# GerHobbelt/ugrep

Hardware: AMD Instinct MI355X
Metric: GB/s scanned + matches/s, 16 GiB synthetic buffer, 1/2/4/8 MI355X (higher is better)
Workload: dtype u8; 1 GPU; 3-literal alternation 'foo|bar|baz' over 16 GiB synthetic ASCII words; config=c2, pattern=foo|bar|baz, bytes_per_gpu=17179869184, total_bytes=17179869184, corpus_kind=1, parallelism=shard1, tables=reference, word=False, dfa_states=9, dfa_row=256, prefilter_ppm=4

## Files before the change

ugrep_amd/csrc/engine.hip:

```cpp
#include <hip/hip_runtime.h>

#include <cstdio>
#include <cstdlib>
#include <cstring>
#include <algorithm>
#include <atomic>
#include <chrono>
#include <condition_variable>
#include <deque>
#include <mutex>
#include <new>
#include <string>
#include <thread>
#include <future>
#include <vector>

#include "../../include/ugpu.h"
#include "plan.hpp"
#include "scan_kernels.hpp"
#include "tables.hpp"

ugpu::Utf8Params utf8_params(const uint8_t* dbuf, uint64_t len)
{
  static std::atomic<int> cached[64];
// ... 73 lines not shown
  bool word = false;
  bool wfast = false;
  bool wu = false;
  bool wforce = false;
  bool xu_exact = false;
  int word_rec = 0;
  bool wxc = false;
  uint32_t bol0 = 1;
  size_t smem = 0;
  size_t xi_smem = 0;
  int xi_rec = 0;
  bool last_xi = false;
  const uint8_t* last_buf = nullptr;
  uint64_t last_args[5] = {0, 0, 0, 0, 0};
  BlockRec* d_recs = nullptr;
  uint64_t* d_entries = nullptr;
  uint64_t* d_obase = nullptr;
  uint16_t* d_inbits = nullptr;
  uint64_t inbits_cap = 0;
  uint64_t* d_fix = nullptr;
  OpenRec* d_open = nullptr;
  uint32_t* d_susp = nullptr;
  SuspRec* d_srec = nullptr;
  DevTotals* d_tot = nullptr;
  uint32_t* d_flags = nullptr;
  DevTotals* h_tot = nullptr;
  uint32_t* h_flags = nullptr;
  hipEvent_t ev0 = nullptr, ev1 = nullptr;
  hipStream_t stream = nullptr;
  ScanParams last{};
  uint64_t off = 0;
  bool have_scan = false;
  bool forest = false;
  uint64_t f_cap = 0;
  uint32_t* d_fex = nullptr;
  uint64_t* d_fvar = nullptr;
  uint64_t* d_fent = nullptr;
  uint64_t* d_fsum = nullptr;
  uint64_t* d_fbase = nullptr;
  bool stage = false, stage_once = false, staged_last = false;
  uint64_t* d_st_start = nullptr;
  uint32_t* d_st_len = nullptr;
  uint32_t* d_st_cap = nullptr;
  uint32_t* d_st_n = nullptr;
};

namespace {

const char* const kBudgetMsg =
    "the FIND chains of this table do not resynchronise on this input (stitch budget exceeded): use the CPU matcher";
// ... 208 lines not shown
  if (pos == 0) pos = fb;
  if (pos > s->f_cap) {
    forest_free(s);
    const uint64_t nb = pos / fb;
    hipError_t e;
    if ((e = hipMalloc(&s->d_fex, pos * 4)) != hipSuccess || (e = hipMalloc(&s->d_fvar, 4 * 8)) != hipSuccess ||
        (e = hipMalloc(&s->d_fent, nb * 8)) != hipSuccess || (e = hipMalloc(&s->d_fsum, nb * 24)) != hipSuccess ||
        (e = hipMalloc(&s->d_fbase, nb * 8)) != hipSuccess) {
      forest_free(s);
      return hip_fail(e, "forest scratch");
    }
    s->f_cap = pos;
  }
  UGPU_TRACE("forest entry %llu hi %llu rend %llu write %d\n", (unsigned long long)entry,
             (unsigned long long)P.hi, (unsigned long long)P.rend, (int)write);
  ForestArgs A{};
  A.ex = s->d_fex;
  A.entry = s->d_fvar;
  A.run = s->d_fvar + 1;
  A.bentry = s->d_fent;
  A.bsum = s->d_fsum;
  A.bbase = s->d_fbase;
  P.flags = s->d_flags;
  HIP_TRY(hipMemsetAsync(s->d_flags, 0, sizeof(uint32_t), st));
  HIP_TRY(launch_forest(P, s->dfa->t.format, A, entry, write, s->d_tot, st));
  HIP_TRY(hipMemcpyAsync(s->h_tot, s->d_tot, sizeof(DevTotals), hipMemcpyDeviceToHost, st));
  HIP_TRY(hipMemcpyAsync(s->h_flags, s->d_flags, sizeof(uint32_t), hipMemcpyDeviceToHost, st));
  HIP_TRY(hipStreamSynchronize(st));
  return UGPU_OK;
}

int dfa_on(const ugpu_dfa* d, int dev, const ugpu_dfa** out);

}

extern "C" {

int ugpu_device_count(int* n)
{
  if (!n) return fail(UGPU_INVAL, "NULL argument");
  *n = 0;
  HIP_TRY(hipGetDeviceCount(n));
  exit_guard_arm();
  return UGPU_OK;
}

// ... 259 lines not shown
      return fail(UGPU_UNSUPPORTED, "tables do not fit in LDS");
    }
    s->word = true;
    s->word_rec = kMaxRec;
    if (const char* env = std::getenv("UGPU_MAX_GRID")) {
      int v = std::atoi(env);
      if (v >= 1 && v <= kMaxRec) s->word_rec = v;
    }
    s->max_rec = s->word_rec;
  }
  if (s->word && dfa->wplus) {
    s->word = false;
    s->wfast = true;
  } else if (s->word && dfa->xcw) {
    s->word = false;
    s->wxc = true;
  }
  if (s->word) {
    HIP_TRY_S(hipMalloc(&s->d_recs, sizeof(BlockRec) * kMaxRec));
    HIP_TRY_S(hipMalloc(&s->d_entries, sizeof(uint64_t) * kMaxRec));
    HIP_TRY_S(hipMalloc(&s->d_obase, sizeof(uint64_t) * kMaxRec));
    HIP_TRY_S(hipMalloc(&s->d_fix, sizeof(uint64_t) * kMaxRec));
    HIP_TRY_S(hipMalloc(&s->d_tot, sizeof(DevTotals)));
    HIP_TRY_S(hipMalloc(&s->d_flags, sizeof(uint32_t)));
    HIP_TRY_S(hipHostMalloc(&s->h_tot, sizeof(DevTotals)));
    HIP_TRY_S(hipHostMalloc(&s->h_flags, sizeof(uint32_t)));
    HIP_TRY_S(hipEventCreate(&s->ev0));
    HIP_TRY_S(hipEventCreate(&s->ev1));
    *out = s;
    return UGPU_OK;
  }
  const char* senv = std::getenv("UGPU_SPARSE");
  s->sparse = (dfa->t.filter || dfa->lb || dfa->wsparse) && dfa->t.format == FMT_BYTE && !(senv && senv[0] == '0');
  s->smem = s->sparse ? sparse_smem_bytes(dfa->ntrans_pad, dfa->t.states, acap_lds_n(dfa))
                      : dense_smem_bytes(dfa->t.format, dfa->ntrans_pad, dfa->t.states);
  if (s->smem > 160 * 1024) {
    delete s;
    return fail(UGPU_UNSUPPORTED, "tables do not fit in LDS");
  }
  int per_cu = 0;
  if (s->sparse) {
    ScanParams probe{};
    HIP_TRY_S(sparse_occupancy(probe, s->smem, &per_cu));
  } else {
    HIP_TRY_S(dense_occupancy(dfa->t.format, dfa->t.cap1 != 0, dfa->d_xtrans != nullptr, s->smem, &per_cu));
  }
  hipDeviceProp_t prop;
  HIP_TRY_S(hipGetDeviceProperties(&prop, s->device));
  if (per_cu < 1) per_cu = 1;
// ... 44 lines not shown
    if (cpc >= 1) {
      s->xc = true;
      s->xu = xu;
      s->wu = wu;
      s->xu_xi = s->xi;
      s->xu_xg = s->xg;
      s->xi = s->xg = false;
      const int cg = prop.multiProcessorCount * cpc * (int)xc_waves();
      s->xi_rec = cg > kMaxRec ? kMaxRec : cg;
      if (const char* env = std::getenv("UGPU_MAX_GRID")) {
        int v = std::atoi(env);
        if (v >= 1 && v <= kMaxRec) s->xi_rec = v;
      }
    }
  }
  HIP_TRY_S(hipMalloc(&s->d_recs, sizeof(BlockRec) * kMaxRec));
  HIP_TRY_S(hipMalloc(&s->d_entries, sizeof(uint64_t) * kMaxRec));
  HIP_TRY_S(hipMalloc(&s->d_obase, sizeof(uint64_t) * kMaxRec));
  HIP_TRY_S(hipMalloc(&s->d_fix, sizeof(uint64_t) * kMaxRec));
  if (s->sparse) {
    HIP_TRY_S(hipMalloc(&s->d_open, sizeof(OpenRec) * kMaxRec));
    HIP_TRY_S(hipMalloc(&s->d_susp, sizeof(uint32_t) * kMaxRec));
    HIP_TRY_S(hipMalloc(&s->d_srec, sizeof(SuspRec) * kMaxRec));
  }
  HIP_TRY_S(hipMalloc(&s->d_tot, sizeof(DevTotals)));
  HIP_TRY_S(hipMalloc(&s->d_flags, sizeof(uint32_t)));
  HIP_TRY_S(hipHostMalloc(&s->h_tot, sizeof(DevTotals)));
  HIP_TRY_S(hipHostMalloc(&s->h_flags, sizeof(uint32_t)));
  HIP_TRY_S(hipEventCreate(&s->ev0));
  HIP_TRY_S(hipEventCreate(&s->ev1));
  *out = s;
  return UGPU_OK;
#undef HIP_TRY_S
}

}

int ugpu_scanner_destroy(ugpu_scanner* s)
{
  if (!s || exiting()) return UGPU_OK;
  (void)hipFree(s->d_recs);
  (void)hipFree(s->d_entries);
  (void)hipFree(s->d_obase);
  (void)hipFree(s->d_inbits);
  (void)hipFree(s->d_fix);
  (void)hipFree(s->d_open);
  (void)hipFree(s->d_susp);
  (void)hipFree(s->d_srec);
  (void)hipFree(s->d_tot);
  (void)hipFree(s->d_flags);
  (void)hipHostFree(s->h_tot);
  (void)hipHostFree(s->h_flags);
  forest_free(s);
  (void)hipFree(s->d_st_start);
  (void)hipFree(s->d_st_len);
  (void)hipFree(s->d_st_cap);
  (void)hipFree(s->d_st_n);
  if (s->ev0) (void)hipEventDestroy(s->ev0);
  if (s->ev1) (void)hipEventDestroy(s->ev1);
  delete s;
  return UGPU_OK;
}

int ugpu_scan(ugpu_scanner* s, const uint8_t* dbuf, uint64_t lo, uint64_t hi, uint64_t read_end, int at_eof,
              uint64_t bias, void* stream)
{
  if (!s || !dbuf) return fail(UGPU_INVAL, "NULL argument");
  if (lo > hi || hi > read_end) return fail(UGPU_INVAL, "need lo <= hi <= read_end");
  hipStream_t st = reinterpret_cast<hipStream_t>(stream);
  if (s->wxc) s->word = false;
  if (s->wfast) {
// ... 12 lines not shown
    }
    s->word = !fast;
  }
  ScanParams P{};
  fill_tables(P, s->dfa);
  P.xu_tab = s->xu ? s->dfa->d_xu : nullptr;
  P.xu_w = s->wu && !s->word ? 1u : 0u;
  P.xu_exact = s->xu_exact ? 1u : 0u;
  P.bol0 = s->bol0;
  if (s->wfast && !s->word) P.wtab = nullptr, P.nwtab = 0;
  geometry_for(P, s, dbuf, lo, hi, read_end, s->off, s->xi || s->xg || s->xc);
  P.delta = (int64_t)bias - (int64_t)s->off;
  P.at_eof = at_eof ? 1u : 0u;
  if (const char* ab = std::getenv("UGPU_ABLATE")) P.ablate = (uint32_t)std::atoi(ab);
  P.recs = s->d_recs;
  P.flags = s->d_flags;
  P.totals = s->d_tot;
  P.entries_out = s->d_entries;
  P.out_base_out = s->d_obase;
  static const bool trunc = env_u64("UGPU_TRUNC", 1) != 0;
  P.open = s->sparse && !P.wtab && !P.acap && trunc ? s->d_open : nullptr;
  P.susp = s->sparse && !P.wtab && !P.acap ? s->d_susp : nullptr;
  P.srec = P.susp ? s->d_srec : nullptr;
  s->staged_last = false;
  if (s->sparse && (s->stage || s->stage_once)) {
    if (!s->d_st_n) {
      const size_t n = (size_t)kMaxRec * kStagePer;
      uint64_t* a = nullptr;
      uint32_t *b = nullptr, *c = nullptr, *d = nullptr;
      hipError_t e = hipMalloc(&a, n * 8);
      if (e == hipSuccess) e = hipMalloc(&b, n * 4);
      if (e == hipSuccess) e = hipMalloc(&c, n * 4);
      if (e == hipSuccess) e = hipMalloc(&d, kMaxRec * 4);
      if (e != hipSuccess) {
        (void)hipFree(a);
        (void)hipFree(b);
        (void)hipFree(c);
        (void)hipFree(d);
        (void)hipGetLastError();
        return fail(UGPU_NOMEM, "staging buffers");
      }
      s->d_st_start = a;
      s->d_st_len = b;
      s->d_st_cap = c;
      s->d_st_n = d;
    }
// ... 2 lines not shown
    P.st_cap = s->d_st_cap;
    P.st_n = s->d_st_n;
    P.st_per = kStagePer;
    s->staged_last = true;
  }
  s->stage_once = false;
  P.inbits = nullptr;
  if (s->pref_write && s->xc && !s->word && !P.xc_w && !P.xu_w && env_u64("UGPU_XC_BITMAP", 1) != 0) {
    const uint64_t need = ((((P.rend + 15) & ~uint64_t(15)) + 2048) >> 3) + 64;
    if (need > s->inbits_cap) {
      (void)hipFree(s->d_inbits);
      s->d_inbits = nullptr;
      s->inbits_cap = 0;
      if (hipMalloc(&s->d_inbits, need + need / 8) == hipSuccess)
        s->inbits_cap = need + need / 8;
      else
        (void)hipGetLastError();
    }
    if (s->d_inbits) P.inbits = s->d_inbits;
  }
  UGPU_TRACE("scan lo %llu hi %llu rend %llu eof %d grid %u xi %d xg %d sparse %d word %d\n", (unsigned long long)P.lo,
             (unsigned long long)P.hi, (unsigned long long)P.rend, at_eof, P.grid, (int)s->xi, (int)s->xg,
             (int)s->sparse, (int)s->word);
  HIP_TRY(hipMemsetAsync(s->d_flags, 0, sizeof(uint32_t), st));
  HIP_TRY(hipEventRecord(s->ev0, st));
  HIP_TRY(launch_main(s, P, false, st, s->xi || s->xg || s->xc));
  HIP_TRY(hipEventRecord(s->ev1, st));
  HIP_TRY(launch_fix(P, s->dfa->t.format, st));
  HIP_TRY(hipMemcpyAsync(s->h_tot, s->d_tot, sizeof(DevTotals), hipMemcpyDeviceToHost, st));
  HIP_TRY(hipMemcpyAsync(s->h_flags, s->d_flags, sizeof(uint32_t), hipMemcpyDeviceToHost, st));
  s->last = P;
  s->last_xi = !s->word && (s->xi || s->xg || s->xc);
  s->last_xc = !s->word && s->xc;
  s->last_buf = dbuf;
  s->last_args[0] = lo;
  s->last_args[1] = hi;
  s->last_args[2] = read_end;
  s->last_args[3] = at_eof ? 1u : 0u;
  s->last_args[4] = bias;
  s->stream = st;
  s->have_scan = true;
  s->forest = false;
  return UGPU_OK;
}

int ugpu_scanner_context(ugpu_scanner* s, int bol0)
{
  if (!s) return fail(UGPU_INVAL, "NULL argument");
  s->bol0 = bol0 ? 1u : 0u;
  return UGPU_OK;
}

int ugpu_scan_totals(ugpu_scanner* s, ugpu_totals* out)
{
  if (!s || !out) return fail(UGPU_INVAL, "NULL argument");
  if (!s->have_scan) return fail(UGPU_INVAL, "no scan issued");
  HIP_TRY(hipStreamSynchronize(s->stream));
  if (s->last_xc && s->xu && (*s->h_flags & UGPU_FLAG_UMIX)) {
    s->xu_exact = true;
    const int rc = ugpu_scan(s, s->last_buf, s->last_args[0], s->last_args[1], s->last_args[2],
                             (int)s->last_args[3], s->last_args[4], s->stream);
    if (rc) return rc;
    HIP_TRY(hipStreamSynchronize(s->stream));
  }
  if (s->wu && !s->word && (*s->h_flags & (UGPU_FLAG_WSLOW | UGPU_FLAG_USLOW))) {
    s->wforce = true;
    const int rc = ugpu_scan(s, s->last_buf, s->last_args[0], s->last_args[1], s->last_args[2],
                             (int)s->last_args[3], s->last_args[4], s->stream);
    s->wforce = false;
    if (rc) return rc;
    HIP_TRY(hipStreamSynchronize(s->stream));
  }
  if (s->wxc && !s->word && (*s->h_flags & UGPU_FLAG_WSLOW)) {
    s->wxc = false;
    s->word = true;
    const int rc = ugpu_scan(s, s->last_buf, s->last_args[0], s->last_args[1], s->last_args[2],
                             (int)s->last_args[3], s->last_args[4], s->stream);
    s->wxc = true;
    if (rc) return rc;
    HIP_TRY(hipStreamSynchronize(s->stream));
// ... 36 lines not shown
  if (!s) return fail(UGPU_INVAL, "NULL argument");
  s->stage = on != 0;
  return UGPU_OK;
}

int ugpu_scan_kernel_ms(ugpu_scanner* s, float* ms)
{
  if (!s || !ms) return fail(UGPU_INVAL, "NULL argument");
  HIP_TRY(hipEventSynchronize(s->ev1));
  HIP_TRY(hipEventElapsedTime(ms, s->ev0, s->ev1));
  return UGPU_OK;
}

int ugpu_scan_offsets(ugpu_scanner* s, uint64_t* d_start, uint32_t* d_len, uint32_t* d_cap, uint64_t capacity,
                      void* stream)
{
  if (!s || !s->have_scan) return fail(UGPU_INVAL, "no scan issued");
  if (!d_cap && (s->dfa->t.cap1 == 0 || s->dfa->t.anchored))
    return fail(UGPU_INVAL, "the table has several accept indices: d_cap is needed");
  hipStream_t st = reinterpret_cast<hipStream_t>(stream);
  HIP_TRY(hipStreamSynchronize(s->stream));
  ScanParams P = s->last;
  bool forest = s->forest || (*s->h_flags & UGPU_FLAG_BUDGET);
  if (s->last_xc && !forest) {
    P.out_base = s->d_obase;
    P.out_start = d_start;
    P.out_len = d_len;
    P.out_cap = d_cap;
    P.out_capacity = capacity;
    P.out_fix = s->d_fix;
    HIP_TRY(hipMemsetAsync(s->d_flags, 0, sizeof(uint32_t), st));
    if (P.inbits)
      HIP_TRY(launch_xc_expand(P, st, s->h_tot->count));
    else
      HIP_TRY(launch_xc(P, true, st, s->h_tot->count));
    HIP_TRY(hipMemcpyAsync(s->h_flags, s->d_flags, sizeof(uint32_t), hipMemcpyDeviceToHost, st));
    HIP_TRY(hipStreamSynchronize(st));
    if (*s->h_flags & UGPU_FLAG_CAPACITY) return fail(UGPU_CAPACITY, "output capacity exceeded");
    if (*s->h_flags & UGPU_FLAG_HALO) return fail(UGPU_HALO, "a match walked past the readable end of the shard");
    return UGPU_OK;
  }
  if (s->last_xi && s->wxc) s->word = true;
  if (s->last_xi && !forest) {
    P = ScanParams{};
    fill_tables(P, s->dfa);
    P.bol0 = s->bol0;
    if (s->wfast) P.wtab = nullptr, P.nwtab = 0;
    uint64_t off = 0;
    geometry_for(P, s, s->last_buf, s->last_args[0], s->last_args[1], s->last_args[2], off, false);
    P.delta = (int64_t)s->last_args[4] - (int64_t)off;
    P.at_eof = (uint32_t)s->last_args[3];
    P.recs = s->d_recs;
    P.flags = s->d_flags;
    P.totals = s->d_tot;
    P.entries_out = s->d_entries;
    P.out_base_out = s->d_obase;
    HIP_TRY(hipMemsetAsync(s->d_flags, 0, sizeof(uint32_t), st));
    HIP_TRY(launch_main(s, P, false, st));
    HIP_TRY(launch_fix(P, s->dfa->t.format, st));
    HIP_TRY(hipMemcpyAsync(s->h_flags, s->d_flags, sizeof(uint32_t), hipMemcpyDeviceToHost, st));
    HIP_TRY(hipStreamSynchronize(st));
    forest = (*s->h_flags & UGPU_FLAG_BUDGET) != 0;
  }
  P.entries = s->d_entries;
  P.out_base = s->d_obase;
  P.out_start = d_start;
  P.out_len = d_len;
  P.out_cap = d_cap;
  P.out_capacity = capacity;
  UGPU_TRACE("offsets forest %d capacity %llu staged %d\n", (int)forest, (unsigned long long)capacity,
             (int)s->staged_last);
  if (!forest && s->staged_last && !s->last_xi) {
    HIP_TRY(hipMemsetAsync(s->d_flags, 0, sizeof(uint32_t), st));
    HIP_TRY(launch_stage_copy(P, st));
    HIP_TRY(hipMemcpyAsync(s->h_flags, s->d_flags, sizeof(uint32_t), hipMemcpyDeviceToHost, st));
    HIP_TRY(hipStreamSynchronize(st));
    s->staged_last = false;
    if (*s->h_flags & UGPU_FLAG_CAPACITY) return fail(UGPU_CAPACITY, "output capacity exceeded");
    if (!(*s->h_flags & UGPU_FLAG_NEEDWRITE)) return UGPU_OK;
  } else {
    P.st_n = nullptr;
  }
  if (!forest) {
    HIP_TRY(hipMemsetAsync(s->d_flags, 0, sizeof(uint32_t), st));
    HIP_TRY(launch_main(s, P, true, st));
    HIP_TRY(hipMemcpyAsync(s->h_flags, s->d_flags, sizeof(uint32_t), hipMemcpyDeviceToHost, st));
    HIP_TRY(hipStreamSynchronize(st));
    forest = (*s->h_flags & UGPU_FLAG_BUDGET) != 0;
  }
  if (forest) {
    const int rc = forest_run(s, P, P.lo, true, st);
    if (rc) return rc;
  }
  if (*s->h_flags & UGPU_FLAG_CAPACITY) return fail(UGPU_CAPACITY, "output capacity exceeded");
  if (*s->h_flags & UGPU_FLAG_HALO) return fail(UGPU_HALO, "a match walked past the readable end of the shard");
  return UGPU_OK;
}

int ugpu_chain_fix(ugpu_scanner* s, const uint8_t* dbuf, uint64_t lo, uint64_t hi, uint64_t read_end, int at_eof,
                   uint64_t bias, uint64_t old_entry, uint64_t new_entry, ugpu_totals* delta, void* stream)
{
  if (!s || !dbuf || !delta) return fail(UGPU_INVAL, "NULL argument");
  hipStream_t st = reinterpret_cast<hipStream_t>(stream);
  ScanParams P{};
  fill_tables(P, s->dfa);
  P.bol0 = s->bol0;
  uint64_t off = 0;
// ... 1924 lines not shown
```

ugrep_amd/csrc/scan_kernels.hip:

```cpp
#include "device_common.hpp"

namespace ugpu {


__device__ __forceinline__ void rec_add(const ScanParams& P, uint64_t b, uint64_t dcnt, uint64_t ddg, uint64_t ddc)
{
  uint64_t* r = reinterpret_cast<uint64_t*>(P.recs + b);
  r[2] += dcnt;
  r[3] += ddg;
  r[4] += ddc;
}

template <int FMT>
__device__ __forceinline__ bool coop_continue(const Tab<FMT>& T, const Win& w, uint32_t& s, uint64_t& q, uint64_t lim,
                                              uint64_t& lastw, uint32_t& lew)
{
  const int lane = threadIdx.x & 63;
  while (q < lim) {
    const uint64_t base = q & ~uint64_t(15);
    const uint64_t sa = base + 16u * (uint32_t)lane;
    uint32_t d[4];
#pragma unroll
    for (int k = 0; k < 4; ++k) {
      uint32_t x = 0;
// ... 273 lines not shown
      if (r[6] == 0 || nx <= c1) {
        met = done = true;
      } else if (e1 != 0) {
        d.put(C, c1, e1 - c1, le1, -1);
        if (nx == e1)
          met = done = true;
        else
          po = e1;
      }
    }
  }
  if (!done)
    met = P.acap   ? merge<FMT, kWalkCtx>(T, w, C, po, nx, bhi, d, ne, ovf, P.merge_budget, &over)
          : P.look ? merge<FMT, kWalkLook>(T, w, C, po, nx, bhi, d, ne, ovf, P.merge_budget, &over)
          : P.wtab ? merge<FMT, kWalkWord>(T, w, C, po, nx, bhi, d, ne, ovf, P.merge_budget, &over)
                   : merge<FMT>(T, w, C, po, nx, bhi, d, ne, ovf, P.merge_budget, &over);
  r[2] += d.cnt;
  r[3] += d.dg;
  r[4] += d.dc;
  exit = ne;
  return met;
}

template <int FMT>
__global__ __launch_bounds__(kFixThreads) void fix_kernel(ScanParams P)
{
  __shared__ uint64_t ent[kMaxRec], exi[kMaxRec];
  __shared__ uint64_t wred[3][kFixThreads / 64];
  __shared__ uint64_t wscan[kFixThreads / 64];
  __shared__ uint32_t openm[kMaxRec / 32];
  constexpr int PER = kMaxRec / kFixThreads;
  const int tid = threadIdx.x, lane = tid & 63, wid = tid >> 6;
  const int G = (int)P.nrec;
  const Tab<FMT> T = tab_global<FMT>(P);
  const Ctx C = P.acap ? Ctx{P.acap, 0u, P.delta} : Ctx{P.caps, P.log_row, P.delta};
  const Win w = win_of(P);
  uint32_t ovf = 0, over = 0;
  const uint32_t fl = __hip_atomic_load(P.flags, __ATOMIC_RELAXED, __HIP_MEMORY_SCOPE_AGENT);
  if (fl & UGPU_FLAG_BUDGET) return;
  const bool any_open = FMT == 0 && P.open && (fl & UGPU_FLAG_OPEN);
  if (any_open)
    for (int i = tid; i < kMaxRec / 32; i += kFixThreads) openm[i] = 0;
  __syncthreads();
#pragma unroll
  for (int j = 0; j < PER; ++j) {
    const int b = j * kFixThreads + tid;
    if (b < G) {
      const uint64_t* r = reinterpret_cast<const uint64_t*>(P.recs + b);
      ent[b] = r[0];
      exi[b] = r[1];
      if (any_open && (r[7] & kRecOpen)) atomicOr(&openm[b >> 5], 1u << (b & 31));
    }
  }
  if (any_open) {
    __syncthreads();
    resolve_open<FMT>(P, T, C, w, G, tid, exi, openm, ovf, over);
    over = __syncthreads_or(over) ? 1u : 0u;
  }
  uint32_t rounds = 0;
  for (;;) {
    __syncthreads();
    uint32_t chm = 0;
#pragma unroll
    for (int j = 0; j < PER; ++j) {
      const int b = j * kFixThreads + tid;
      if (b > 0 && b < G && exi[b - 1] != ent[b]) chm |= 1u << j;
    }
    __syncthreads();
    for (uint32_t m = chm; m;) {
      const int j = __builtin_ctz(m);
      m &= m - 1;
      const uint64_t b = (uint64_t)j * kFixThreads + tid;
      const uint64_t nx = exi[b - 1];
      if (nx == ent[b]) continue;
      uint64_t tb = P.t0 + b * P.tpb;
      uint64_t te = tb + P.tpb < P.t1 ? tb + P.tpb : P.t1;
      if (tb > te) tb = te;
      const uint64_t bhi = clampu(te * P.unit, P.lo, P.hi);
      uint64_t ne = 0;
      if (!fix_block<FMT>(P, T, C, w, b, ent[b], nx, bhi, ne, ovf, over)) exi[b] = ne;
      ent[b] = nx;
    }
    if (!__syncthreads_or(chm != 0)) break;
    if (__syncthreads_or(over) || ++rounds >= P.max_rounds) {
      over = 1;
      break;
    }
  }
  __threadfence_block();
  __syncthreads();
  uint64_t cnt[PER];
  uint64_t md = 0, mdc = 0;
#pragma unroll
  for (int j = 0; j < PER; ++j) {
    const int b = j * kFixThreads + tid;
    cnt[j] = 0;
    if (b < G) {
      const uint64_t* r = reinterpret_cast<const uint64_t*>(P.recs + b);
      cnt[j] = r[2];
      md += r[3];
      mdc += r[4];
    }
  }
  const uint64_t sd = wave_sum(md), sdc = wave_sum(mdc);
  if (lane == 0) {
    wred[1][wid] = sd;
    wred[2][wid] = sdc;
  }
  uint64_t carry = 0;
#pragma unroll
  for (int j = 0; j < PER; ++j) {
    uint64_t incl = cnt[j];
#pragma unroll
    for (int o = 1; o < 64; o <<= 1) {
      uint64_t y = __shfl_up(incl, o, 64);
      if (lane >= o) incl += y;
    }
    __syncthreads();
    if (lane == 63) wscan[wid] = incl;
    __syncthreads();
    uint64_t off = carry, tot = 0;
    for (int k = 0; k < kFixThreads / 64; ++k) {
      if (k < wid) off += wscan[k];
      tot += wscan[k];
    }
    const int b = j * kFixThreads + tid;
    if (b < G) {
      P.out_base_out[b] = off + incl - cnt[j];
      P.entries_out[b] = ent[b];
    }
    carry += tot;
  }
  if (ovf) atomicOr(P.flags, UGPU_FLAG_HALO);
  if (over && tid == 0) atomicOr(P.flags, UGPU_FLAG_BUDGET);
  __syncthreads();
  if (tid == 0) {
    uint64_t d = 0, e = 0;
    for (int k = 0; k < kFixThreads / 64; ++k) {
      d += wred[1][k];
      e += wred[2][k];
    }
    const uint64_t c = carry;
    DevTotals* t = P.totals;
    t->count = c;
    t->digest = d;
    t->dcap = e;
    t->entry = ent[0];
    t->exit = exi[G - 1];
    t->rounds = rounds;
  }
}

template <int FMT>
__global__ void chain_fix_kernel(ScanParams P, uint64_t old_entry, uint64_t new_entry)
{
  if (threadIdx.x != 0 || blockIdx.x != 0) return;
  const Tab<FMT> T = tab_global<FMT>(P);
  const Ctx C = P.acap ? Ctx{P.acap, 0u, P.delta} : Ctx{P.caps, P.log_row, P.delta};
  const Win w = win_of(P);
  uint32_t ovf = 0, over = 0;
  CountEm d;
  uint64_t ne = 0;
  bool met = P.acap   ? merge<FMT, kWalkCtx>(T, w, C, old_entry, new_entry, P.hi, d, ne, ovf, P.merge_budget, &over)
             : P.look ? merge<FMT, kWalkLook>(T, w, C, old_entry, new_entry, P.hi, d, ne, ovf, P.merge_budget, &over)
             : P.wtab ? merge<FMT, kWalkWord>(T, w, C, old_entry, new_entry, P.hi, d, ne, ovf, P.merge_budget, &over)
                      : merge<FMT>(T, w, C, old_entry, new_entry, P.hi, d, ne, ovf, P.merge_budget, &over);
  DevTotals* t = P.totals;
  t->count = d.cnt;
  t->digest = d.dg;
  t->dcap = d.dc;
  t->entry = new_entry;
  t->exit = met ? ~0ull : ne;
// ... 74 lines not shown
```

ugrep_amd/csrc/scan_kernels.hpp:

```cpp
#pragma once
#include <hip/hip_runtime.h>
#include <cstdint>

namespace ugpu {

constexpr int kMaxRec = 8192;
constexpr int kFixThreads = 1024;
constexpr int kWaveTile = 4096;
constexpr int kSpWaves = 4;
#ifndef UGPU_DSEG_BYTE
#define UGPU_DSEG_BYTE 188
#endif
#ifndef UGPU_DSEG_CLASS
#define UGPU_DSEG_CLASS 92
#endif
#ifndef UGPU_DWAVES_BYTE
#define UGPU_DWAVES_BYTE 4
#endif
#ifndef UGPU_DWAVES_CLASS
#define UGPU_DWAVES_CLASS 8
#endif
constexpr int kDSegByte = UGPU_DSEG_BYTE;
constexpr int kDSegClass = UGPU_DSEG_CLASS;
constexpr int kDWavesByte = UGPU_DWAVES_BYTE;
// ... 109 lines not shown
  uint32_t xc_w;
  uint32_t xu_w;
  uint32_t xu_exact;
  const uint8_t* xu_tab;
  const uint32_t* xu_bm3;
  uint32_t xu_null;
  uint16_t* inbits;
  const uint32_t* acap;
  uint32_t wstart;
  uint32_t ft2;
  const uint32_t* lb_cls;
  const uint32_t* dom;
  const uint32_t* look;
  uint32_t dom_all;
  uint32_t bol0;
  uint32_t nul;
  uint32_t ctx_word;
  uint32_t acap_n;
  const uint32_t* amap;
  uint32_t acap_lds;
  OpenRec* open;
  uint32_t* susp;
  SuspRec* srec;
};

struct ForestArgs {
  uint64_t c_lo, c_hi;
  uint32_t nblk;
  uint32_t* ex;
  uint64_t* entry;
  uint64_t* run;
  uint64_t* bentry;
  uint64_t* bsum;
  uint64_t* bbase;
};
constexpr uint64_t kFChunk = 64ull << 20;
hipError_t launch_forest(const ScanParams& P, uint32_t format, const ForestArgs& A, uint64_t entry, bool write,
                         DevTotals* tot, hipStream_t stream);
uint64_t forest_block();

hipError_t launch_fix(const ScanParams& P, uint32_t format, hipStream_t stream);
hipError_t launch_pack_records(const uint64_t* start, const uint32_t* len, const uint32_t* cap, uint64_t n,
                               uint64_t base, uint8_t* out, int caps, int dense, uint64_t* esc, uint32_t* nesc,
                               hipStream_t stream);
hipError_t launch_chain_fix(const ScanParams& P, uint32_t format, uint64_t old_entry, uint64_t new_entry,
                            hipStream_t stream);
// ... 98 lines not shown
```

ugrep_amd/csrc/sparse_kernel.hip:

```cpp
#include "device_common.hpp"

#ifndef UGPU_SP_CTX_OCC
#define UGPU_SP_CTX_OCC 4
#endif
#ifndef UGPU_SP_CTX_WIN
#define UGPU_SP_CTX_WIN 1
#endif

namespace ugpu {

namespace {

struct FTab {
  uint32_t t0lo, t0hi, t1lo, t1hi, t2;
};

template <bool FT2>
__device__ __forceinline__ uint32_t bucket_bits(uint32_t x, const FTab& F)
{
  const uint32_t r0 = __builtin_amdgcn_perm(F.t0hi, F.t0lo, x & 0x07070707u);
  const uint32_t r1 = __builtin_amdgcn_perm(F.t1hi, F.t1lo, (x >> 3) & 0x07070707u);
  if constexpr (FT2) return r0 & r1;
  const uint32_t r2 = __builtin_amdgcn_perm(F.t2, F.t2, (x >> 6) & 0x03030303u);
  return r0 & r1 & r2;
// ... 597 lines not shown
      uint32_t m = mk, r = rank;
      while (m) {
        const uint32_t bit = __builtin_ctz(m);
        m &= m - 1;
        if (r - done < take) dl[w.dn + r - done] = p0 + bit;
        ++r;
      }
      w.dn += take;
      done += take;
    }
  }
}

__device__ __forceinline__ TileLoad wave_tile(const uint8_t* wbase, uint32_t i, uint32_t rel)
{
  const uint32_t off = i * (uint32_t)kWaveTile;
  const uint32_t n = rel > off ? rel - off : 0u;
  const int nr = __builtin_amdgcn_readfirstlane((int)(n < (uint32_t)kWaveTile ? n : (uint32_t)kWaveTile));
  return TileLoad{__builtin_amdgcn_make_buffer_rsrc(const_cast<uint8_t*>(wbase + off), (short)0, nr, 0x00020000)};
}

}

template <bool WRITE, int ABL, int W = kWalkPlain, bool STAGE = false, bool RESUME = false, bool LB = false,
          bool FT2 = false>
__global__ __launch_bounds__(kSpWaves * 64, RESUME ? 1 : (W == kWalkCtx ? UGPU_SP_CTX_OCC : 6)) void sparse_kernel(ScanParams P)
{
  extern __shared__ __attribute__((aligned(16))) uint8_t smem[];
  const int tid = threadIdx.x, lane = tid & 63;
  const int wid = __builtin_amdgcn_readfirstlane(tid >> 6);
  const uint64_t gw = (uint64_t)blockIdx.x * kSpWaves + wid;
  bool mine = true;
  if constexpr (RESUME) {
    mine = P.susp[gw] != 0;
    if (!__syncthreads_or(mine)) return;
  }
  uint8_t* aux = smem + wid * kAux;
  uint64_t* dl = reinterpret_cast<uint64_t*>(aux);
  uint8_t* scr = aux;
  uint16_t* ltrans = reinterpret_cast<uint16_t*>(smem + kSpWaves * kAux);
  uint32_t* lcaps = reinterpret_cast<uint32_t*>(ltrans + P.ntrans_pad);
  {
    const uint4* src = reinterpret_cast<const uint4*>(P.trans);
    uint4* dst = reinterpret_cast<uint4*>(ltrans);
    for (uint32_t i = tid; i < P.ntrans_pad / 8; i += kSpWaves * 64) dst[i] = src[i];
    for (uint32_t i = tid; i < P.nstates; i += kSpWaves * 64) lcaps[i] = P.caps[i];
    if constexpr (W == kWalkCtx) {
      if (P.acap_lds) {
        uint32_t* la = lcaps + P.nstates;
        for (uint32_t i = tid; i < P.acap_n; i += kSpWaves * 64) la[i] = P.acap[i];
        if (P.ctx_word)
          for (uint32_t i = tid; i < P.nstates; i += kSpWaves * 64) la[P.acap_n + i] = P.amap[i];
      }
    }
  }
  __syncthreads();
  if (!mine) return;
  const Tab<0> T{ltrans, nullptr, P.start, P.accb};
  const Ctx C = W == kWalkCtx ? Ctx{P.acap_lds ? lcaps + P.nstates : P.acap, 0u, P.delta}
                              : Ctx{lcaps, P.log_row, P.delta};
  const FTab F{P.ft[0], P.ft[1], P.ft[2], P.ft[3], P.ft[4]};

  uint64_t tb = P.t0 + gw * P.tpb;
  uint64_t te = tb + P.tpb < P.t1 ? tb + P.tpb : P.t1;
  if (tb > te) tb = te;
  const uint64_t wlo = clampu(tb * kWaveTile, P.lo, P.hi);
  const uint64_t whi = clampu(te * kWaveTile, P.lo, P.hi);
  WaveChain w;
  w.x = WRITE ? P.entries[gw] : wlo;
  w.dn = 0;
  w.widx = WRITE ? P.out_base[gw] : 0;
  w.wover = 0;
  w.ovf = 0;
  w.first = w.open = 0;
  w.c1 = w.e1 = 0;
  w.le1 = 0;
  w.pend = 0;
  w.rs = w.ptile = 0;
  w.wlo = wlo;
  w.whi = whi;
// ... 120 lines not shown
        const uint64_t c = wave_sum(w.acc.cnt), d = wave_sum(w.acc.dg), dc = wave_sum(w.acc.dc);
        if (lane == 0) {
          SuspRec* sr = P.srec + gw;
          sr->x = w.x;
          sr->widx = w.widx;
          sr->cnt = c;
          sr->dg = d;
          sr->dc = dc;
          sr->c1 = w.c1;
          sr->e1 = w.e1;
          sr->rs = w.rs;
          sr->lbr = w.lbr;
          sr->lbs = w.lbs;
          sr->sgn = w.sg.n;
          sr->wover = w.wover;
          sr->ovf = w.ovf;
          sr->first = w.first;
          sr->open = w.open;
          sr->le1 = w.le1;
          sr->sgover = w.sg.over;
          sr->tile = (uint32_t)((w.ptile - wb) / kWaveTile);
          sr->dn = 0;
          P.susp[gw] = 1;
        }
        return;
      }
      if (lane == 0) P.susp[gw] = 0;
    }
  }
  uint64_t x = w.x > whi ? w.x : whi;
  if (tb == te) x = wlo;
  if (w.open) x = lim;

  if (w.ovf) atomicOr(P.flags, UGPU_FLAG_HALO);
  if (!WRITE && w.open && lane == 0) atomicOr(P.flags, UGPU_FLAG_OPEN);
  if (w.wover) atomicOr(P.flags, UGPU_FLAG_CAPACITY);
  if constexpr (!WRITE) {
    const uint64_t c = wave_sum(w.acc.cnt), d = wave_sum(w.acc.dg), dc = wave_sum(w.acc.dc);
    if (STAGE && lane == 0) P.st_n[gw] = w.sg.over ? kStageOver : (uint32_t)w.sg.n;
    if (lane == 0) {
      BlockRec rec;
      rec.entry = wlo;
      rec.exit = x;
      rec.cnt = c;
      rec.dg = d;
      rec.dc = dc;
      rec.pad0 = rec.pad1 = rec.pad2 = 0;
      if (W == kWalkPlain) {
        rec.pad0 = w.c1;
        rec.pad1 = w.first ? w.e1 : 0;
        rec.pad2 = (uint64_t)w.le1 | (w.open ? kRecOpen : 0) | kRecFirst;
      }
      P.recs[gw] = rec;
    }
  }
}

size_t sparse_smem_bytes(uint32_t ntrans_pad, uint32_t nstates, uint32_t nlds_acap)
{
  size_t b = (size_t)kSpWaves * kAux + 2 * (size_t)ntrans_pad + 4 * (size_t)nstates + 4 * (size_t)nlds_acap;
  return (b + 15) & ~size_t(15);
}

namespace {

template <bool WRITE, int ABL, int W = kWalkPlain, bool STAGE = false, bool RESUME = false, bool LB = false,
          bool FT2 = false>
hipError_t sparse_launch(const ScanParams& P, size_t smem, hipStream_t stream)
{
  static size_t attr_smem = 65536;
  if (smem > attr_smem) {
    hipError_t e =
        hipFuncSetAttribute(reinterpret_cast<const void*>(&sparse_kernel<WRITE, ABL, W, STAGE, RESUME, LB, FT2>),
                            hipFuncAttributeMaxDynamicSharedMemorySize, (int)smem);
    if (e != hipSuccess) return e;
    attr_smem = smem;
  }
  hipLaunchKernelGGL((sparse_kernel<WRITE, ABL, W, STAGE, RESUME, LB, FT2>), dim3(P.grid), dim3(kSpWaves * 64), smem,
                     stream, P);
  return hipGetLastError();
}

template <bool WRITE, int ABL, int W = kWalkPlain, bool STAGE = false, bool LB = false, bool FT2 = false>
hipError_t sparse_one(const ScanParams& P, size_t smem, hipStream_t stream)
{
  hipError_t e = sparse_launch<WRITE, ABL, W, STAGE, false, LB, FT2>(P, smem, stream);
  if constexpr (W == kWalkPlain && ABL == 0) {
    if (e == hipSuccess && P.susp) e = sparse_launch<WRITE, 0, kWalkPlain, STAGE, true, LB, FT2>(P, smem, stream);
  }
  return e;
}

__global__ __launch_bounds__(256) void stage_copy_kernel(ScanParams P)
{
  const uint32_t b = blockIdx.x;
  if (b >= P.nrec) return;
  const uint32_t n = P.st_n[b];
  const uint64_t base = P.out_base[b];
  const uint64_t next = b + 1 < P.nrec ? P.out_base[b + 1] : P.totals->count;
  const bool ok = n != kStageOver && P.entries[b] == P.recs[b].entry && next - base == n;
  __syncthreads();
// ... 76 lines not shown
```

Measured before the change: 6417 GB/s.

## Compact resume launch via suspend list and publish totals to pinned host memory

Suspended waves now append their id to a device list through an atomic counter, and the resume kernel runs over that compact list with a smaller grid instead of launching a full grid where most blocks exit early. The fix kernel writes totals and flags straight into mapped pinned host memory and clears the device flags itself, which removes the two D2H memcpys and the per-scan memset. It also reads the record counts in the first pass, re-reading only if they could have changed, and replaces the serialized per-chunk block scan with a single two-level scan. The changes add system-scope fences and zero-copy host writes, and rely on the flags-clean state being tracked correctly across streams and the error paths.

New measurement: 6452 GB/s (median of 6 runs). No clear change (+0.5%).

```diff
diff --git a/ugrep_amd/csrc/engine.hip b/ugrep_amd/csrc/engine.hip
--- a/ugrep_amd/csrc/engine.hip
+++ b/ugrep_amd/csrc/engine.hip
@@ -119,10 +119,15 @@
   OpenRec* d_open = nullptr;
   uint32_t* d_susp = nullptr;
   SuspRec* d_srec = nullptr;
+  uint32_t* d_susp_list = nullptr;
+  uint32_t resume_grid = 0;
   DevTotals* d_tot = nullptr;
   uint32_t* d_flags = nullptr;
   DevTotals* h_tot = nullptr;
   uint32_t* h_flags = nullptr;
+  DevTotals* dh_tot = nullptr;
+  uint32_t* dh_flags = nullptr;
+  bool flags_clean = false;
   hipEvent_t ev0 = nullptr, ev1 = nullptr;
   hipStream_t stream = nullptr;
   ScanParams last{};
@@ -377,6 +382,7 @@
   A.bsum = s->d_fsum;
   A.bbase = s->d_fbase;
   P.flags = s->d_flags;
+  s->flags_clean = false;
   HIP_TRY(hipMemsetAsync(s->d_flags, 0, sizeof(uint32_t), st));
   HIP_TRY(launch_forest(P, s->dfa->t.format, A, entry, write, s->d_tot, st));
   HIP_TRY(hipMemcpyAsync(s->h_tot, s->d_tot, sizeof(DevTotals), hipMemcpyDeviceToHost, st));
@@ -682,9 +688,11 @@
     HIP_TRY_S(hipMalloc(&s->d_obase, sizeof(uint64_t) * kMaxRec));
     HIP_TRY_S(hipMalloc(&s->d_fix, sizeof(uint64_t) * kMaxRec));
     HIP_TRY_S(hipMalloc(&s->d_tot, sizeof(DevTotals)));
-    HIP_TRY_S(hipMalloc(&s->d_flags, sizeof(uint32_t)));
+    HIP_TRY_S(hipMalloc(&s->d_flags, 2 * sizeof(uint32_t)));
     HIP_TRY_S(hipHostMalloc(&s->h_tot, sizeof(DevTotals)));
     HIP_TRY_S(hipHostMalloc(&s->h_flags, sizeof(uint32_t)));
+    HIP_TRY_S(hipHostGetDevicePointer(reinterpret_cast<void**>(&s->dh_tot), s->h_tot, 0));
+    HIP_TRY_S(hipHostGetDevicePointer(reinterpret_cast<void**>(&s->dh_flags), s->h_flags, 0));
     HIP_TRY_S(hipEventCreate(&s->ev0));
     HIP_TRY_S(hipEventCreate(&s->ev1));
     *out = s;
@@ -775,11 +783,17 @@
     HIP_TRY_S(hipMalloc(&s->d_open, sizeof(OpenRec) * kMaxRec));
     HIP_TRY_S(hipMalloc(&s->d_susp, sizeof(uint32_t) * kMaxRec));
     HIP_TRY_S(hipMalloc(&s->d_srec, sizeof(SuspRec) * kMaxRec));
+    HIP_TRY_S(hipMalloc(&s->d_susp_list, sizeof(uint32_t) * kMaxRec));
+    s->resume_grid = (uint32_t)((s->max_rec + kSpWaves - 1) / kSpWaves);
+    const uint64_t rg = env_u64("UGPU_RESUME_GRID", 0);
+    if (rg >= 1 && rg < s->resume_grid) s->resume_grid = (uint32_t)rg;
   }
   HIP_TRY_S(hipMalloc(&s->d_tot, sizeof(DevTotals)));
-  HIP_TRY_S(hipMalloc(&s->d_flags, sizeof(uint32_t)));
+  HIP_TRY_S(hipMalloc(&s->d_flags, 2 * sizeof(uint32_t)));
   HIP_TRY_S(hipHostMalloc(&s->h_tot, sizeof(DevTotals)));
   HIP_TRY_S(hipHostMalloc(&s->h_flags, sizeof(uint32_t)));
+  HIP_TRY_S(hipHostGetDevicePointer(reinterpret_cast<void**>(&s->dh_tot), s->h_tot, 0));
+  HIP_TRY_S(hipHostGetDevicePointer(reinterpret_cast<void**>(&s->dh_flags), s->h_flags, 0));
   HIP_TRY_S(hipEventCreate(&s->ev0));
   HIP_TRY_S(hipEventCreate(&s->ev1));
   *out = s;
@@ -800,6 +814,7 @@
   (void)hipFree(s->d_open);
   (void)hipFree(s->d_susp);
   (void)hipFree(s->d_srec);
+  (void)hipFree(s->d_susp_list);
   (void)hipFree(s->d_tot);
   (void)hipFree(s->d_flags);
   (void)hipHostFree(s->h_tot);
@@ -858,6 +873,11 @@
   P.open = s->sparse && !P.wtab && !P.acap && trunc ? s->d_open : nullptr;
   P.susp = s->sparse && !P.wtab && !P.acap ? s->d_susp : nullptr;
   P.srec = P.susp ? s->d_srec : nullptr;
+  P.nsusp = s->d_flags + 1;
+  P.susp_list = P.susp ? s->d_susp_list : nullptr;
+  P.resume_grid = s->resume_grid;
+  P.host_totals = s->dh_tot;
+  P.host_flags = s->dh_flags;
   s->staged_last = false;
   if (s->sparse && (s->stage || s->stage_once)) {
     if (!s->d_st_n) {
@@ -906,13 +926,14 @@
   UGPU_TRACE("scan lo %llu hi %llu rend %llu eof %d grid %u xi %d xg %d sparse %d word %d\n", (unsigned long long)P.lo,
              (unsigned long long)P.hi, (unsigned long long)P.rend, at_eof, P.grid, (int)s->xi, (int)s->xg,
              (int)s->sparse, (int)s->word);
-  HIP_TRY(hipMemsetAsync(s->d_flags, 0, sizeof(uint32_t), st));
+  const bool clean = s->flags_clean && st == s->stream;
+  s->flags_clean = false;
+  if (!clean) HIP_TRY(hipMemsetAsync(s->d_flags, 0, 2 * sizeof(uint32_t), st));
   HIP_TRY(hipEventRecord(s->ev0, st));
   HIP_TRY(launch_main(s, P, false, st, s->xi || s->xg || s->xc));
   HIP_TRY(hipEventRecord(s->ev1, st));
   HIP_TRY(launch_fix(P, s->dfa->t.format, st));
-  HIP_TRY(hipMemcpyAsync(s->h_tot, s->d_tot, sizeof(DevTotals), hipMemcpyDeviceToHost, st));
-  HIP_TRY(hipMemcpyAsync(s->h_flags, s->d_flags, sizeof(uint32_t), hipMemcpyDeviceToHost, st));
+  s->flags_clean = true;
   s->last = P;
   s->last_xi = !s->word && (s->xi || s->xg || s->xc);
   s->last_xc = !s->word && s->xc;
@@ -939,7 +960,10 @@
 {
   if (!s || !out) return fail(UGPU_INVAL, "NULL argument");
   if (!s->have_scan) return fail(UGPU_INVAL, "no scan issued");
-  HIP_TRY(hipStreamSynchronize(s->stream));
+  if (const hipError_t e = hipStreamSynchronize(s->stream); e != hipSuccess) {
+    s->flags_clean = false;
+    return hip_fail(e, "hipStreamSynchronize(s->stream)");
+  }
   if (s->last_xc && s->xu && (*s->h_flags & UGPU_FLAG_UMIX)) {
     s->xu_exact = true;
     const int rc = ugpu_scan(s, s->last_buf, s->last_args[0], s->last_args[1], s->last_args[2],
@@ -1022,6 +1046,7 @@
   HIP_TRY(hipStreamSynchronize(s->stream));
   ScanParams P = s->last;
   bool forest = s->forest || (*s->h_flags & UGPU_FLAG_BUDGET);
+  s->flags_clean = false;
   if (s->last_xc && !forest) {
     P.out_base = s->d_obase;
     P.out_start = d_start;
@@ -1055,10 +1080,11 @@
     P.totals = s->d_tot;
     P.entries_out = s->d_entries;
     P.out_base_out = s->d_obase;
-    HIP_TRY(hipMemsetAsync(s->d_flags, 0, sizeof(uint32_t), st));
+    P.nsusp = s->d_flags + 1;
+    P.host_flags = s->dh_flags;
+    HIP_TRY(hipMemsetAsync(s->d_flags, 0, 2 * sizeof(uint32_t), st));
     HIP_TRY(launch_main(s, P, false, st));
     HIP_TRY(launch_fix(P, s->dfa->t.format, st));
-    HIP_TRY(hipMemcpyAsync(s->h_flags, s->d_flags, sizeof(uint32_t), hipMemcpyDeviceToHost, st));
     HIP_TRY(hipStreamSynchronize(st));
     forest = (*s->h_flags & UGPU_FLAG_BUDGET) != 0;
   }
@@ -1082,7 +1108,7 @@
     P.st_n = nullptr;
   }
   if (!forest) {
-    HIP_TRY(hipMemsetAsync(s->d_flags, 0, sizeof(uint32_t), st));
+    HIP_TRY(hipMemsetAsync(s->d_flags, 0, 2 * sizeof(uint32_t), st));
     HIP_TRY(launch_main(s, P, true, st));
     HIP_TRY(hipMemcpyAsync(s->h_flags, s->d_flags, sizeof(uint32_t), hipMemcpyDeviceToHost, st));
     HIP_TRY(hipStreamSynchronize(st));
diff --git a/ugrep_amd/csrc/scan_kernels.hip b/ugrep_amd/csrc/scan_kernels.hip
--- a/ugrep_amd/csrc/scan_kernels.hip
+++ b/ugrep_amd/csrc/scan_kernels.hip
@@ -319,12 +319,21 @@
   return met;
 }
 
+__device__ __forceinline__ void publish_flags(const ScanParams& P, uint32_t f)
+{
+  if (P.host_flags) *P.host_flags = f;
+  __hip_atomic_store(P.flags, 0u, __ATOMIC_RELAXED, __HIP_MEMORY_SCOPE_AGENT);
+  if (P.nsusp) *P.nsusp = 0;
+  __threadfence_system();
+}
+
 template <int FMT>
 __global__ __launch_bounds__(kFixThreads) void fix_kernel(ScanParams P)
 {
   __shared__ uint64_t ent[kMaxRec], exi[kMaxRec];
   __shared__ uint64_t wred[3][kFixThreads / 64];
   __shared__ uint64_t wscan[kFixThreads / 64];
+  __shared__ uint64_t wpart[kMaxRec / 64];
   __shared__ uint32_t openm[kMaxRec / 32];
   constexpr int PER = kMaxRec / kFixThreads;
   const int tid = threadIdx.x, lane = tid & 63, wid = tid >> 6;
@@ -334,21 +343,31 @@
   const Win w = win_of(P);
   uint32_t ovf = 0, over = 0;
   const uint32_t fl = __hip_atomic_load(P.flags, __ATOMIC_RELAXED, __HIP_MEMORY_SCOPE_AGENT);
-  if (fl & UGPU_FLAG_BUDGET) return;
   const bool any_open = FMT == 0 && P.open && (fl & UGPU_FLAG_OPEN);
   if (any_open)
     for (int i = tid; i < kMaxRec / 32; i += kFixThreads) openm[i] = 0;
   __syncthreads();
+  if (fl & UGPU_FLAG_BUDGET) {
+    if (tid == 0) publish_flags(P, fl);
+    return;
+  }
+  uint64_t cnt[PER];
+  uint64_t md = 0, mdc = 0;
 #pragma unroll
   for (int j = 0; j < PER; ++j) {
     const int b = j * kFixThreads + tid;
+    cnt[j] = 0;
     if (b < G) {
       const uint64_t* r = reinterpret_cast<const uint64_t*>(P.recs + b);
       ent[b] = r[0];
       exi[b] = r[1];
+      cnt[j] = r[2];
+      md += r[3];
+      mdc += r[4];
       if (any_open && (r[7] & kRecOpen)) atomicOr(&openm[b >> 5], 1u << (b & 31));
     }
   }
+  bool reread = any_open;
   if (any_open) {
     __syncthreads();
     resolve_open<FMT>(P, T, C, w, G, tid, exi, openm, ovf, over);
@@ -379,6 +398,7 @@
       ent[b] = nx;
     }
     if (!__syncthreads_or(chm != 0)) break;
+    reread = true;
     if (__syncthreads_or(over) || ++rounds >= P.max_rounds) {
       over = 1;
       break;
@@ -386,17 +406,18 @@
   }
   __threadfence_block();
   __syncthreads();
-  uint64_t cnt[PER];
-  uint64_t md = 0, mdc = 0;
-#pragma unroll
-  for (int j = 0; j < PER; ++j) {
-    const int b = j * kFixThreads + tid;
-    cnt[j] = 0;
-    if (b < G) {
-      const uint64_t* r = reinterpret_cast<const uint64_t*>(P.recs + b);
-      cnt[j] = r[2];
-      md += r[3];
-      mdc += r[4];
+  if (reread) {
+    md = mdc = 0;
+#pragma unroll
+    for (int j = 0; j < PER; ++j) {
+      const int b = j * kFixThreads + tid;
+      cnt[j] = 0;
+      if (b < G) {
+        const uint64_t* r = reinterpret_cast<const uint64_t*>(P.recs + b);
+        cnt[j] = r[2];
+        md += r[3];
+        mdc += r[4];
+      }
     }
   }
   const uint64_t sd = wave_sum(md), sdc = wave_sum(mdc);
@@ -404,30 +425,42 @@
     wred[1][wid] = sd;
     wred[2][wid] = sdc;
   }
-  uint64_t carry = 0;
+  constexpr int kFixWaves = kFixThreads / 64;
+  static_assert(PER * kFixWaves == 128, "wave 0 scans two wave sums per lane");
+  uint64_t incl[PER];
 #pragma unroll
   for (int j = 0; j < PER; ++j) {
-    uint64_t incl = cnt[j];
+    incl[j] = cnt[j];
 #pragma unroll
     for (int o = 1; o < 64; o <<= 1) {
-      uint64_t y = __shfl_up(incl, o, 64);
-      if (lane >= o) incl += y;
-    }
-    __syncthreads();
-    if (lane == 63) wscan[wid] = incl;
-    __syncthreads();
-    uint64_t off = carry, tot = 0;
-    for (int k = 0; k < kFixThreads / 64; ++k) {
-      if (k < wid) off += wscan[k];
-      tot += wscan[k];
-    }
+      uint64_t y = __shfl_up(incl[j], o, 64);
+      if (lane >= o) incl[j] += y;
+    }
+    if (lane == 63) wpart[j * kFixWaves + wid] = incl[j];
+  }
+  __syncthreads();
+  if (wid == 0) {
+    const uint64_t v0 = wpart[2 * lane], v1 = wpart[2 * lane + 1];
+    uint64_t is = v0 + v1;
+#pragma unroll
+    for (int o = 1; o < 64; o <<= 1) {
+      uint64_t y = __shfl_up(is, o, 64);
+      if (lane >= o) is += y;
+    }
+    wpart[2 * lane] = is - v0 - v1;
+    wpart[2 * lane + 1] = is - v1;
+    if (lane == 63) wscan[0] = is;
+  }
+  __syncthreads();
+#pragma unroll
+  for (int j = 0; j < PER; ++j) {
     const int b = j * kFixThreads + tid;
     if (b < G) {
-      P.out_base_out[b] = off + incl - cnt[j];
+      P.out_base_out[b] = wpart[j * kFixWaves + wid] + incl[j] - cnt[j];
       P.entries_out[b] = ent[b];
     }
-    carry += tot;
-  }
+  }
+  const uint64_t carry = wscan[0];
   if (ovf) atomicOr(P.flags, UGPU_FLAG_HALO);
   if (over && tid == 0) atomicOr(P.flags, UGPU_FLAG_BUDGET);
   __syncthreads();
@@ -437,14 +470,18 @@
       d += wred[1][k];
       e += wred[2][k];
     }
-    const uint64_t c = carry;
-    DevTotals* t = P.totals;
-    t->count = c;
-    t->digest = d;
-    t->dcap = e;
-    t->entry = ent[0];
-    t->exit = exi[G - 1];
-    t->rounds = rounds;
+    const uint32_t f = __hip_atomic_load(P.flags, __ATOMIC_RELAXED, __HIP_MEMORY_SCOPE_AGENT);
+    DevTotals t;
+    t.count = carry;
+    t.digest = d;
+    t.dcap = e;
+    t.entry = ent[0];
+    t.exit = exi[G - 1];
+    t.flags = f;
+    t.rounds = rounds;
+    *P.totals = t;
+    if (P.host_totals) *P.host_totals = t;
+    publish_flags(P, f);
   }
 }
 
diff --git a/ugrep_amd/csrc/scan_kernels.hpp b/ugrep_amd/csrc/scan_kernels.hpp
--- a/ugrep_amd/csrc/scan_kernels.hpp
+++ b/ugrep_amd/csrc/scan_kernels.hpp
@@ -155,6 +155,11 @@
   OpenRec* open;
   uint32_t* susp;
   SuspRec* srec;
+  uint32_t* nsusp;
+  uint32_t* susp_list;
+  uint32_t resume_grid;
+  DevTotals* host_totals;
+  uint32_t* host_flags;
 };
 
 struct ForestArgs {
diff --git a/ugrep_amd/csrc/sparse_kernel.hip b/ugrep_amd/csrc/sparse_kernel.hip
--- a/ugrep_amd/csrc/sparse_kernel.hip
+++ b/ugrep_amd/csrc/sparse_kernel.hip
@@ -643,40 +643,10 @@
 
 }
 
-template <bool WRITE, int ABL, int W = kWalkPlain, bool STAGE = false, bool RESUME = false, bool LB = false,
-          bool FT2 = false>
-__global__ __launch_bounds__(kSpWaves * 64, RESUME ? 1 : (W == kWalkCtx ? UGPU_SP_CTX_OCC : 6)) void sparse_kernel(ScanParams P)
-{
-  extern __shared__ __attribute__((aligned(16))) uint8_t smem[];
-  const int tid = threadIdx.x, lane = tid & 63;
-  const int wid = __builtin_amdgcn_readfirstlane(tid >> 6);
-  const uint64_t gw = (uint64_t)blockIdx.x * kSpWaves + wid;
-  bool mine = true;
-  if constexpr (RESUME) {
-    mine = P.susp[gw] != 0;
-    if (!__syncthreads_or(mine)) return;
-  }
-  uint8_t* aux = smem + wid * kAux;
-  uint64_t* dl = reinterpret_cast<uint64_t*>(aux);
-  uint8_t* scr = aux;
-  uint16_t* ltrans = reinterpret_cast<uint16_t*>(smem + kSpWaves * kAux);
-  uint32_t* lcaps = reinterpret_cast<uint32_t*>(ltrans + P.ntrans_pad);
-  {
-    const uint4* src = reinterpret_cast<const uint4*>(P.trans);
-    uint4* dst = reinterpret_cast<uint4*>(ltrans);
-    for (uint32_t i = tid; i < P.ntrans_pad / 8; i += kSpWaves * 64) dst[i] = src[i];
-    for (uint32_t i = tid; i < P.nstates; i += kSpWaves * 64) lcaps[i] = P.caps[i];
-    if constexpr (W == kWalkCtx) {
-      if (P.acap_lds) {
-        uint32_t* la = lcaps + P.nstates;
-        for (uint32_t i = tid; i < P.acap_n; i += kSpWaves * 64) la[i] = P.acap[i];
-        if (P.ctx_word)
-          for (uint32_t i = tid; i < P.nstates; i += kSpWaves * 64) la[P.acap_n + i] = P.amap[i];
-      }
-    }
-  }
-  __syncthreads();
-  if (!mine) return;
+template <bool WRITE, int ABL, int W, bool STAGE, bool RESUME, bool LB, bool FT2>
+__device__ __forceinline__ void sparse_wave(const ScanParams& P, const uint64_t gw, const int lane, uint64_t* dl,
+                                            uint8_t* scr, const uint16_t* ltrans, const uint32_t* lcaps)
+{
   const Tab<0> T{ltrans, nullptr, P.start, P.accb};
   const Ctx C = W == kWalkCtx ? Ctx{P.acap_lds ? lcaps + P.nstates : P.acap, 0u, P.delta}
                               : Ctx{lcaps, P.log_row, P.delta};
@@ -843,6 +813,8 @@
           sr->tile = (uint32_t)((w.ptile - wb) / kWaveTile);
           sr->dn = 0;
           P.susp[gw] = 1;
+          const uint32_t slot = atomicAdd(P.nsusp, 1u);
+          if (slot < P.nrec) P.susp_list[slot] = (uint32_t)gw;
         }
         return;
       }
@@ -877,6 +849,52 @@
   }
 }
 
+template <bool WRITE, int ABL, int W = kWalkPlain, bool STAGE = false, bool RESUME = false, bool LB = false,
+          bool FT2 = false>
+__global__ __launch_bounds__(kSpWaves * 64, RESUME ? 4 : (W == kWalkCtx ? UGPU_SP_CTX_OCC : 6)) void sparse_kernel(ScanParams P)
+{
+  extern __shared__ __attribute__((aligned(16))) uint8_t smem[];
+  const int tid = threadIdx.x, lane = tid & 63;
+  const int wid = __builtin_amdgcn_readfirstlane(tid >> 6);
+  uint32_t nsu = 0;
+  if constexpr (RESUME) {
+    nsu = *P.nsusp;
+    if (nsu > P.nrec) nsu = P.nrec;
+    if (blockIdx.x * (uint32_t)kSpWaves >= nsu) return;
+  }
+  uint8_t* aux = smem + wid * kAux;
+  uint64_t* dl = reinterpret_cast<uint64_t*>(aux);
+  uint8_t* scr = aux;
+  uint16_t* ltrans = reinterpret_cast<uint16_t*>(smem + kSpWaves * kAux);
+  uint32_t* lcaps = reinterpret_cast<uint32_t*>(ltrans + P.ntrans_pad);
+  {
+    const uint4* src = reinterpret_cast<const uint4*>(P.trans);
+    uint4* dst = reinterpret_cast<uint4*>(ltrans);
+    for (uint32_t i = tid; i < P.ntrans_pad / 8; i += kSpWaves * 64) dst[i] = src[i];
+    for (uint32_t i = tid; i < P.nstates; i += kSpWaves * 64) lcaps[i] = P.caps[i];
+    if constexpr (W == kWalkCtx) {
+      if (P.acap_lds) {
+        uint32_t* la = lcaps + P.nstates;
+        for (uint32_t i = tid; i < P.acap_n; i += kSpWaves * 64) la[i] = P.acap[i];
+        if (P.ctx_word)
+          for (uint32_t i = tid; i < P.nstates; i += kSpWaves * 64) la[P.acap_n + i] = P.amap[i];
+      }
+    }
+  }
+  __syncthreads();
+  if constexpr (RESUME) {
+    for (uint32_t k = blockIdx.x * (uint32_t)kSpWaves + (uint32_t)wid; k < nsu; k += gridDim.x * (uint32_t)kSpWaves) {
+      const uint32_t gw = (uint32_t)__builtin_amdgcn_readfirstlane((int)P.susp_list[k]);
+      if (gw >= P.nrec) continue;
+      wave_lds_sync();
+      sparse_wave<WRITE, ABL, W, STAGE, RESUME, LB, FT2>(P, gw, lane, dl, scr, ltrans, lcaps);
+    }
+  } else {
+    sparse_wave<WRITE, ABL, W, STAGE, RESUME, LB, FT2>(P, (uint64_t)blockIdx.x * kSpWaves + wid, lane, dl, scr, ltrans,
+                                                       lcaps);
+  }
+}
+
 size_t sparse_smem_bytes(uint32_t ntrans_pad, uint32_t nstates, uint32_t nlds_acap)
 {
   size_t b = (size_t)kSpWaves * kAux + 2 * (size_t)ntrans_pad + 4 * (size_t)nstates + 4 * (size_t)nlds_acap;
@@ -897,7 +915,9 @@
     if (e != hipSuccess) return e;
     attr_smem = smem;
   }
-  hipLaunchKernelGGL((sparse_kernel<WRITE, ABL, W, STAGE, RESUME, LB, FT2>), dim3(P.grid), dim3(kSpWaves * 64), smem,
+  uint32_t grid = P.grid;
+  if (RESUME && P.resume_grid && P.resume_grid < grid) grid = P.resume_grid;
+  hipLaunchKernelGGL((sparse_kernel<WRITE, ABL, W, STAGE, RESUME, LB, FT2>), dim3(grid), dim3(kSpWaves * 64), smem,
                      stream, P);
   return hipGetLastError();
 }
```
